# nv-tlabs/GEN3C

Measured on NVIDIA H100. Metric: denoise-steps/sec, 7B DiT, 121-frame 720p latent, higher is better.
Workload: dtype bf16

## Files before the change

gen3c_b200/csrc/attn_wgmma.cu:

```cuda
#include <cmath>
#include <cstdlib>

#include "kernels.h"

namespace g3c {

constexpr int ATT_THREADS = 384;
constexpr int ATT_TILE = ATT_ROWS_PER_CTA;
constexpr int ATT_HALF_BYTES = 128 * 128;
constexpr int ATT_TILE_BYTES = 2 * ATT_HALF_BYTES;
constexpr int ATT_STAGES = 2;
constexpr int ATT_SMEM = ATT_TILE_BYTES + ATT_STAGES * 2 * ATT_TILE_BYTES + 256 + 1024;
static_assert(ATT_SMEM <= 227 * 1024, "attention: Q + K/V rings exceed the 227 KB of shared memory per block");
static_assert(1 + 4 * ATT_STAGES + 3 <= 256 / 8, "attention: barriers exceed their 256-byte area");
static_assert(ATT_STAGES == 2, "attention: the consumer loop is unrolled for a ring depth of 2");
constexpr float ATT_RESCALE_LOG2 = 8.0f;

struct AttnParams {
  int Lq, Lk, heads;
  int ldo;
  int vt_chunk_len;
  __nv_bfloat16* O;
  float scale_log2;
  const uint32_t* chunk_flags;
  uint32_t flag_seq;
  int first_chunk;
  unsigned long long peer_timeout_ns;
  unsigned long long* wait_ns;
  unsigned long long* trace;
};

static unsigned long long* g_attn_trace = nullptr;

#define ATT_TR(role, slot)                                                                                  \
  do {                                                                                                      \
    if constexpr (kTrace) {                                                                                 \
      if (blockIdx.x == 0 && blockIdx.y == 0 && j < 64 && (threadIdx.x % 128) == 0)                         \
        p.trace[((role) * 64 + j) * 8 + (slot)] = clock64();                                                \
    }                                                                                                       \
  } while (0)

__device__ __forceinline__ float ex2_approx(float x) {
  float y;
  asm("ex2.approx.ftz.f32 %0, %1;\n" : "=f"(y) : "f"(x));
  return y;
}

__device__ __forceinline__ bool softmax_tile(float (&s)[64], float (&m_ref)[2], float (&l_run)[2], float (&alpha)[2],
                                             float sl2) {
  float mx[2] = {-INFINITY, -INFINITY};
#pragma unroll
  for (int i = 0; i < 16; ++i) {
    mx[0] = fmaxf(mx[0], fmaxf(s[4 * i], s[4 * i + 1]));
    mx[1] = fmaxf(mx[1], fmaxf(s[4 * i + 2], s[4 * i + 3]));
  }
#pragma unroll
  for (int h = 0; h < 2; ++h) {
    mx[h] = fmaxf(mx[h], __shfl_xor_sync(0xffffffffu, mx[h], 1));
    mx[h] = fmaxf(mx[h], __shfl_xor_sync(0xffffffffu, mx[h], 2));
    mx[h] *= sl2;
  }
  const bool keep = __all_sync(0xffffffffu, mx[0] - m_ref[0] <= ATT_RESCALE_LOG2 && mx[1] - m_ref[1] <= ATT_RESCALE_LOG2);
  if (!keep) {
#pragma unroll
    for (int h = 0; h < 2; ++h) {
      const float nm = fmaxf(m_ref[h], mx[h]);
      alpha[h] = ex2_approx(m_ref[h] - nm);
      m_ref[h] = nm;
      l_run[h] *= alpha[h];
    }
  }
  const float nm0 = -m_ref[0], nm1 = -m_ref[1];
#pragma unroll
  for (int i = 0; i < 16; ++i) {
    s[4 * i] = ex2_approx(fmaf(s[4 * i], sl2, nm0));
    s[4 * i + 1] = ex2_approx(fmaf(s[4 * i + 1], sl2, nm0));
    s[4 * i + 2] = ex2_approx(fmaf(s[4 * i + 2], sl2, nm1));
    s[4 * i + 3] = ex2_approx(fmaf(s[4 * i + 3], sl2, nm1));
    l_run[0] += s[4 * i] + s[4 * i + 1];
    l_run[1] += s[4 * i + 2] + s[4 * i + 3];
  }
  return !keep;
}

constexpr uint32_t ATT_SDESC_HI = (1024u >> 4) | (1u << 30);
__device__ __forceinline__ uint64_t sdesc_at(uint32_t lo, uint32_t bytes) {
  return (static_cast<uint64_t>(ATT_SDESC_HI) << 32) | (lo + (bytes >> 4));
}

__device__ __forceinline__ void issue_s(float (&s)[64], uint32_t dq, uint32_t dk) {
#pragma unroll
  for (int kk = 0; kk < 8; ++kk) {
    const uint32_t off = (kk >> 2) * ATT_HALF_BYTES + (kk & 3) * 32;
    wgmma_ss_n128(s, sdesc_at(dq, off), sdesc_at(dk, off), kk > 0 ? 1u : 0u);
  }
}

template <bool kVTokenMajor>
__device__ __forceinline__ void issue_pv(float (&o)[64], const uint32_t (&pa)[32], uint32_t dv) {
#pragma unroll
  for (int kk = 0; kk < 8; ++kk) {
    const uint32_t a[4] = {pa[4 * kk], pa[4 * kk + 1], pa[4 * kk + 2], pa[4 * kk + 3]};
    if constexpr (kVTokenMajor)
      wgmma_rs_n128_tb(o, a, sdesc_at(dv, kk * 16 * 128));
    else
      wgmma_rs_n128(o, a, sdesc_at(dv, (kk >> 2) * ATT_HALF_BYTES + (kk & 3) * 32));
  }
}

__device__ __forceinline__ void mask_key_tail(float (&s)[64], int valid, uint32_t lane) {
#pragma unroll
  for (int i = 0; i < 16; ++i) {
    const int col = 8 * i + 2 * (int)(lane % 4);
    if (col >= valid) s[4 * i] = s[4 * i + 2] = -INFINITY;
    if (col + 1 >= valid) s[4 * i + 1] = s[4 * i + 3] = -INFINITY;
  }
}

__device__ __forceinline__ void pack_p(uint32_t (&pa)[32], const float (&s)[64]) {
#pragma unroll
  for (int i = 0; i < 16; ++i) {
    pa[2 * i] = pack_bf16x2(s[4 * i], s[4 * i + 1]);
    pa[2 * i + 1] = pack_bf16x2(s[4 * i + 2], s[4 * i + 3]);
  }
}

template <bool kTrace, bool kVTokenMajor = false>
__global__ void __launch_bounds__(ATT_THREADS, 1)
    k_attn_fwd(const __grid_constant__ CUtensorMap tmQ, const __grid_constant__ CUtensorMap tmK,
               const __grid_constant__ CUtensorMap tmV, const AttnParams p) {
  extern __shared__ uint8_t smem_raw[];
  uint8_t* smem = reinterpret_cast<uint8_t*>((reinterpret_cast<uintptr_t>(smem_raw) + 1023) &
                                             ~static_cast<uintptr_t>(1023));
  uint8_t* smem_q = smem;
  uint8_t* smem_k = smem + ATT_TILE_BYTES;
  uint8_t* smem_v = smem_k + ATT_STAGES * ATT_TILE_BYTES;
  uint64_t* bars = reinterpret_cast<uint64_t*>(smem_v + ATT_STAGES * ATT_TILE_BYTES);
  uint64_t* q_full = bars;
  uint64_t* k_full = bars + 1;
  uint64_t* v_full = k_full + ATT_STAGES;
  uint64_t* k_empty = v_full + ATT_STAGES;
  uint64_t* v_empty = k_empty + ATT_STAGES;
  uint64_t* turn = v_empty + ATT_STAGES;
  uint64_t* done = turn + 2;

  const uint32_t wg = threadIdx.x / 128;
  const uint32_t tid = threadIdx.x % 128;
  const int head = blockIdx.y;
  const int q0 = blockIdx.x * ATT_TILE;
  const int n_kv = kVTokenMajor ? (p.Lk + ATT_TILE - 1) / ATT_TILE : p.Lk / ATT_TILE;

  if (threadIdx.x == 0) {
    tma_prefetch_desc(&tmQ);
    tma_prefetch_desc(&tmK);
    tma_prefetch_desc(&tmV);
    mbar_init(q_full, 1);
    for (int i = 0; i < ATT_STAGES; ++i) {
      mbar_init(&k_full[i], 1);
      mbar_init(&v_full[i], 1);
      mbar_init(&k_empty[i], 2);
      mbar_init(&v_empty[i], 2);
    }
    for (int c = 0; c < 2; ++c) mbar_init(&turn[c], 4);
    for (int w = 0; w < 4; ++w) mbar_arrive(&turn[0]);
    mbar_init(done, 2);
    fence_barrier_init();
  }
  __syncthreads();

  if (wg == 0) {
    setmaxnreg_dec<24>();
    if (tid == 0) {
      mbar_expect_tx(q_full, ATT_TILE_BYTES);
      for (int h = 0; h < 2; ++h) tma_load_2d(smem_q + h * ATT_HALF_BYTES, &tmQ, q_full, head * 128 + h * 64, q0);
      const int tiles_per_chunk = p.vt_chunk_len / ATT_TILE;
      const int n_chunks = p.Lk / p.vt_chunk_len;
      uint32_t stage = 0, phase = 0;
      for (int j = 0; j < n_kv; ++j) {
        int chunk = 0, within = j;
        if constexpr (!kVTokenMajor) {
          chunk = p.first_chunk + j / tiles_per_chunk;
          if (chunk >= n_chunks) chunk -= n_chunks;
          within = j % tiles_per_chunk;
          if (p.chunk_flags && within == 0 && chunk != p.first_chunk) {
            uint32_t v, spins = 0;
            uint64_t t0 = 0;
            for (;;) {
              asm volatile("ld.acquire.sys.global.u32 %0, [%1];\n" : "=r"(v) : "l"(p.chunk_flags + chunk) : "memory");
              if ((int)(v - p.flag_seq) >= 0) break;
              if (t0 == 0) t0 = global_timer_ns();
              if ((++spins & 0x3FFu) == 0 && global_timer_ns() - t0 > p.peer_timeout_ns) asm volatile("trap;\n");
            }
            if (t0 != 0 && p.wait_ns) atomicAdd(p.wait_ns, (unsigned long long)(global_timer_ns() - t0));
            asm volatile("fence.proxy.async.global;\n" ::: "memory");
          }
        }
        const int kv0 = chunk * p.vt_chunk_len + within * ATT_TILE;
        mbar_wait_ns(&k_empty[stage], phase ^ 1, p.peer_timeout_ns);
        mbar_expect_tx(&k_full[stage], ATT_TILE_BYTES);
        for (int h = 0; h < 2; ++h)
          tma_load_2d(smem_k + stage * ATT_TILE_BYTES + h * ATT_HALF_BYTES, &tmK, &k_full[stage], head * 128 + h * 64,
                      kv0);
        mbar_wait_ns(&v_empty[stage], phase ^ 1, p.peer_timeout_ns);
        mbar_expect_tx(&v_full[stage], ATT_TILE_BYTES);
        for (int h = 0; h < 2; ++h) {
          if constexpr (kVTokenMajor)
            tma_load_2d(smem_v + stage * ATT_TILE_BYTES + h * ATT_HALF_BYTES, &tmV, &v_full[stage],
                        head * 128 + h * 64, kv0);
          else
            tma_load_3d(smem_v + stage * ATT_TILE_BYTES + h * ATT_HALF_BYTES, &tmV, &v_full[stage],
                        within * ATT_TILE + h * 64, head * 128, chunk);
        }
        if (++stage == ATT_STAGES) {
          stage = 0;
          phase ^= 1;
        }
      }
      mbar_wait_ns(done, 0, p.peer_timeout_ns);
    }
  } else {
    setmaxnreg_inc<240>();
    const uint32_t c = __shfl_sync(0xffffffffu, wg - 1, 0);
    const uint32_t warp = tid / 32, lane = tid % 32;
    const unsigned long long tmo = p.peer_timeout_ns;
    float o[64];
#pragma unroll
    for (int i = 0; i < 64; ++i) o[i] = 0.f;
    float s[64];
    uint32_t pa[32];
    float m_ref[2] = {-INFINITY, -INFINITY};
    float l_run[2] = {0.f, 0.f};
    float alpha[2];
    const float sl2 = p.scale_log2;
    const uint32_t dq = (uint32_t)make_sdesc_sw128(smem_u32(smem_q + c * 64 * 128));
    uint32_t dk[ATT_STAGES], dv[ATT_STAGES];
#pragma unroll
    for (int st = 0; st < ATT_STAGES; ++st) {
      dk[st] = (uint32_t)make_sdesc_sw128(smem_u32(smem_k + st * ATT_TILE_BYTES));
      dv[st] = (uint32_t)(kVTokenMajor ? make_sdesc_sw128_mn(smem_u32(smem_v + st * ATT_TILE_BYTES), ATT_HALF_BYTES)
                                       : make_sdesc_sw128(smem_u32(smem_v + st * ATT_TILE_BYTES)));
    }
    int j = 0;
    mbar_wait_ns_or_exit(q_full, 0, tmo);
    mbar_wait_ns_or_exit(&k_full[0], 0, tmo);
    mbar_wait_ns_or_exit(&turn[c], 0, tmo);
    ATT_TR(1 + c, 0);
    wgmma_fence();
    issue_s(s, dq, dk[0]);
    wgmma_commit();
    if (lane == 0) mbar_arrive(&turn[c ^ 1]);
    ATT_TR(1 + c, 1);
    wgmma_wait<0>();
    fence_regs(s);
    if (tid == 0) mbar_arrive(&k_empty[0]);
    ATT_TR(1 + c, 2);
    if constexpr (kVTokenMajor) {
      if (n_kv == 1) mask_key_tail(s, p.Lk, lane);
    }
    softmax_tile(s, m_ref, l_run, alpha, sl2);
    pack_p(pa, s);
    ATT_TR(1 + c, 3);
    auto step = [&](int kst, int vst, uint32_t kpar, uint32_t vpar, int valid) {
      mbar_wait_ns_or_exit(&k_full[kst], kpar, tmo);
      mbar_wait_ns_or_exit(&v_full[vst], vpar, tmo);
      mbar_wait_ns_or_exit(&turn[c], (uint32_t)j & 1u, tmo);
      ATT_TR(1 + c, 0);
      wgmma_fence();
      issue_s(s, dq, kst ? dk[1] : dk[0]);
      wgmma_commit();
      issue_pv<kVTokenMajor>(o, pa, vst ? dv[1] : dv[0]);
      wgmma_commit();
      if (lane == 0) mbar_arrive(&turn[c ^ 1]);
      ATT_TR(1 + c, 1);
      wgmma_wait<1>();
      fence_regs(s);
      if (tid == 0) mbar_arrive(&k_empty[kst]);
      ATT_TR(1 + c, 2);
      if (valid < ATT_TILE) mask_key_tail(s, valid, lane);
      const bool rescale = softmax_tile(s, m_ref, l_run, alpha, sl2);
      ATT_TR(1 + c, 3);
      wgmma_wait<0>();
      fence_regs(o);
      fence_regs(pa);
      if (tid == 0) mbar_arrive(&v_empty[vst]);
      ATT_TR(1 + c, 4);
      if (rescale) {
#pragma unroll
        for (int i = 0; i < 16; ++i) {
          o[4 * i] *= alpha[0];
          o[4 * i + 1] *= alpha[0];
          o[4 * i + 2] *= alpha[1];
          o[4 * i + 3] *= alpha[1];
        }
      }
      pack_p(pa, s);
    };
    const int j_end = kVTokenMajor ? n_kv - 1 : n_kv;
    uint32_t ph = 0;
    for (j = 1; j < j_end; ++j) {
      step(1, 0, ph, ph, ATT_TILE);
      if (++j == j_end) break;
      step(0, 1, ph ^ 1u, ph, ATT_TILE);
      ph ^= 1u;
    }
    if constexpr (kVTokenMajor) {
      if (n_kv > 1) {
        j = n_kv - 1;
        step(j & 1, (j - 1) & 1, ((uint32_t)j >> 1) & 1u, ((uint32_t)(j - 1) >> 1) & 1u, p.Lk - j * ATT_TILE);
      }
      j = n_kv;
    }
    const int vst = (n_kv - 1) & 1;
    mbar_wait_ns_or_exit(&v_full[vst], ((uint32_t)(n_kv - 1) >> 1) & 1u, tmo);
    mbar_wait_ns_or_exit(&turn[c], (uint32_t)n_kv & 1u, tmo);
    ATT_TR(1 + c, 0);
    wgmma_fence();
    issue_pv<kVTokenMajor>(o, pa, vst ? dv[1] : dv[0]);
    wgmma_commit();
    if (lane == 0) mbar_arrive(&turn[c ^ 1]);
    ATT_TR(1 + c, 1);
    wgmma_wait<0>();
    fence_regs(o);
    fence_regs(pa);
    if (tid == 0) mbar_arrive(&v_empty[vst]);
    ATT_TR(1 + c, 4);
    float inv[2];
#pragma unroll
    for (int h = 0; h < 2; ++h) {
      float l = l_run[h];
      l += __shfl_xor_sync(0xffffffffu, l, 1);
      l += __shfl_xor_sync(0xffffffffu, l, 2);
      inv[h] = 1.0f / l;
    }
    const int row_a = q0 + (int)(c * 64 + warp * 16 + lane / 4);
#pragma unroll
    for (int h = 0; h < 2; ++h) {
      const int row = row_a + 8 * h;
      if (row >= p.Lq) continue;
      __nv_bfloat16* dst = p.O + (size_t)row * p.ldo + head * 128 + 2 * (lane % 4);
#pragma unroll
      for (int i = 0; i < 16; ++i)
        *reinterpret_cast<uint32_t*>(dst + 8 * i) = pack_bf16x2(o[4 * i + 2 * h] * inv[h], o[4 * i + 2 * h + 1] * inv[h]);
    }
    if (tid == 0) mbar_arrive(done);
  }
}

static int make_tmap_tokens(CUtensorMap* m, const void* base, int rows, int heads, int ld) {
  uint64_t dims[2] = {(uint64_t)heads * 128, (uint64_t)rows}, str[1] = {(uint64_t)ld * 2};
  uint32_t box[2] = {64, 128};
  return make_tmap_bf16_sw128(m, base, 2, dims, str, box);
}

static float scale_log2(float scale) {
  const float s = scale * 1.4426950408889634f;
  return fabsf(s - 1.0f) < 1e-6f ? 1.0f : s;
}

int attn_fwd(const void* q, const void* k, const void* vt, void* o, int Lq, int Lk, int heads,
             int ldq, int ldk, int ldo, int vt_chunk_len, float scale, cudaStream_t st, const ChunkGate* gate) {
  G3C_REQUIRE(q && k && vt && o, "attn: null operand");
  G3C_REQUIRE(Lq > 0 && Lk > 0 && heads > 0, "attn: bad sizes");
  G3C_REQUIRE(Lk % ATT_TILE == 0, "attn: Lk=%d must be a multiple of 128", Lk);
  if (vt_chunk_len <= 0) vt_chunk_len = Lk;
  G3C_REQUIRE(Lk % vt_chunk_len == 0 && vt_chunk_len % ATT_TILE == 0,
              "attn: vt_chunk_len=%d must divide Lk=%d and be a multiple of 128", vt_chunk_len, Lk);
  G3C_REQUIRE(ldq % 8 == 0 && ldk % 8 == 0 && ldo % 8 == 0 && ldq >= heads * 128 &&
                  ldk >= heads * 128 && ldo >= heads * 128,
              "attn: leading dimensions must be >= heads*128 and multiples of 8");
  G3C_REQUIRE((reinterpret_cast<uintptr_t>(o) & 15) == 0, "attn: O must be 16-byte aligned");
  CUtensorMap tmQ, tmK, tmV;
  int rc = make_tmap_tokens(&tmQ, q, Lq, heads, ldq);
  if (rc) return rc;
  rc = make_tmap_tokens(&tmK, k, Lk, heads, ldk);
  if (rc) return rc;
  {
    const int chunks = Lk / vt_chunk_len;
    uint64_t dims[3] = {(uint64_t)vt_chunk_len, (uint64_t)heads * 128, (uint64_t)chunks};
    uint64_t str[2] = {(uint64_t)vt_chunk_len * 2, (uint64_t)vt_chunk_len * 2 * heads * 128};
    uint32_t box[3] = {64, 128, 1};
    rc = make_tmap_bf16_sw128(&tmV, vt, 3, dims, str, box);
    if (rc) return rc;
  }
  static bool configured = false;
  if (!configured) {
    G3C_CUDA(cudaFuncSetAttribute(k_attn_fwd<false>, cudaFuncAttributeMaxDynamicSharedMemorySize, ATT_SMEM));
    G3C_CUDA(cudaFuncSetAttribute(k_attn_fwd<true>, cudaFuncAttributeMaxDynamicSharedMemorySize, ATT_SMEM));
    configured = true;
  }
  AttnParams p;
  p.Lq = Lq;
  p.Lk = Lk;
  p.heads = heads;
  p.ldo = ldo;
  p.vt_chunk_len = vt_chunk_len;
  p.O = reinterpret_cast<__nv_bfloat16*>(o);
  p.scale_log2 = scale_log2(scale);
  p.chunk_flags = gate ? gate->flags : nullptr;
  p.peer_timeout_ns = gate ? peer_timeout_ns() : G3C_MBAR_TIMEOUT_NS;
  p.wait_ns = gate ? gate->wait_ns : nullptr;
  p.flag_seq = gate ? gate->seq : 0;
  p.first_chunk = gate ? gate->first : 0;
  p.trace = g_attn_trace;
  G3C_REQUIRE(p.first_chunk >= 0 && p.first_chunk < Lk / vt_chunk_len, "attn: first chunk %d out of range", p.first_chunk);
  dim3 grid((Lq + ATT_TILE - 1) / ATT_TILE, heads);
  if (g_attn_trace) k_attn_fwd<true><<<grid, ATT_THREADS, ATT_SMEM, st>>>(tmQ, tmK, tmV, p);
  else k_attn_fwd<false><<<grid, ATT_THREADS, ATT_SMEM, st>>>(tmQ, tmK, tmV, p);
  G3C_CUDA(cudaGetLastError());
  return G3C_OK;
}

int attn_fwd_sbhd(const void* q, const void* k, const void* v, void* o, int Lq, int Lk, int batch, int heads, int ldq,
                  int ldk, int ldv, int ldo, float scale, cudaStream_t st) {
  G3C_REQUIRE(q && k && v && o, "attn_sbhd: null operand");
  G3C_REQUIRE(Lq > 0 && Lk > 0, "attn_sbhd: Lq=%d and Lk=%d must be >= 1", Lq, Lk);
  G3C_REQUIRE(batch > 0 && heads > 0 && (long long)batch * heads <= 65535,
              "attn_sbhd: batch=%d x heads=%d must be in [1, 65535]", batch, heads);
  const int bh = batch * heads;
  G3C_REQUIRE(ldq % 8 == 0 && ldk % 8 == 0 && ldv % 8 == 0 && ldo % 8 == 0 && ldq >= bh * 128 && ldk >= bh * 128 &&
                  ldv >= bh * 128 && ldo >= bh * 128,
              "attn_sbhd: leading dimensions (%d, %d, %d, %d) must be >= batch*heads*128 = %d and multiples of 8", ldq,
              ldk, ldv, ldo, bh * 128);
  G3C_REQUIRE(((reinterpret_cast<uintptr_t>(q) | reinterpret_cast<uintptr_t>(k) | reinterpret_cast<uintptr_t>(v) |
                reinterpret_cast<uintptr_t>(o)) & 15) == 0,
              "attn_sbhd: q, k, v and o must be 16-byte aligned");
  CUtensorMap tmQ, tmK, tmV;
  int rc = make_tmap_tokens(&tmQ, q, Lq, bh, ldq);
  if (rc) return rc;
  rc = make_tmap_tokens(&tmK, k, Lk, bh, ldk);
  if (rc) return rc;
  rc = make_tmap_tokens(&tmV, v, Lk, bh, ldv);
  if (rc) return rc;
  static bool configured = false;
  if (!configured) {
    G3C_CUDA(cudaFuncSetAttribute(k_attn_fwd<false, true>, cudaFuncAttributeMaxDynamicSharedMemorySize, ATT_SMEM));
    configured = true;
  }
  AttnParams p = {};
  p.Lq = Lq;
  p.Lk = Lk;
  p.heads = bh;
  p.ldo = ldo;
  p.vt_chunk_len = Lk;
  p.O = reinterpret_cast<__nv_bfloat16*>(o);
  p.scale_log2 = scale_log2(scale);
  p.peer_timeout_ns = G3C_MBAR_TIMEOUT_NS;
  dim3 grid((Lq + ATT_TILE - 1) / ATT_TILE, bh);
  k_attn_fwd<false, true><<<grid, ATT_THREADS, ATT_SMEM, st>>>(tmQ, tmK, tmV, p);
  G3C_CUDA(cudaGetLastError());
  return G3C_OK;
}

}

extern "C" int g3c_attn_set_trace(unsigned long long* device_buffer) {
  g3c::g_attn_trace = device_buffer;
  return G3C_OK;
}

extern "C" int g3c_attn_fwd(const void* q, const void* k, const void* vt, void* o, int Lq, int Lk,
                            int heads, int ldq, int ldk, int ldo, int vt_chunk_len, float scale,
                            void* stream) {
  return g3c::attn_fwd(q, k, vt, o, Lq, Lk, heads, ldq, ldk, ldo, vt_chunk_len, scale,
                       (cudaStream_t)stream, nullptr);
}

extern "C" int g3c_attn_fwd_gated(const void* q, const void* k, const void* vt, void* o, int Lq, int Lk, int heads,
                                  int ldq, int ldk, int ldo, int vt_chunk_len, float scale, const uint32_t* flags,
                                  uint32_t seq, int first, unsigned long long* wait_ns, void* stream) {
  g3c::ChunkGate gate;
  gate.flags = flags;
  gate.seq = seq;
  gate.first = first;
  gate.wait_ns = wait_ns;
  return g3c::attn_fwd(q, k, vt, o, Lq, Lk, heads, ldq, ldk, ldo, vt_chunk_len, scale, (cudaStream_t)stream, &gate);
}

extern "C" int g3c_attn_fwd_sbhd(const void* q, const void* k, const void* v, void* o, int Lq, int Lk, int batch,
                                 int heads, int ldq, int ldk, int ldv, int ldo, float scale, void* stream) {
  return g3c::attn_fwd_sbhd(q, k, v, o, Lq, Lk, batch, heads, ldq, ldk, ldv, ldo, scale, (cudaStream_t)stream);
}
```

gen3c_b200/csrc/common.cuh:

```cuda
#pragma once
#include <cuda.h>
#include <cuda_bf16.h>
#include <cuda_runtime.h>
#include <stdint.h>
#include <stdio.h>

#include "../../include/gen3c_b200.h"
#include "wgmma_ops.cuh"

namespace g3c {

void set_error(const char* fmt, ...);
int cuda_fail(cudaError_t e, const char* what, const char* file, int line);
#define G3C_CUDA(x)                                                         \
  do {                                                                      \
    cudaError_t _e = (x);                                                   \
    if (_e != cudaSuccess) return ::g3c::cuda_fail(_e, #x, __FILE__, __LINE__); \
  } while (0)
#define G3C_REQUIRE(cond, ...)        \
  do {                                \
    if (!(cond)) {                    \
      ::g3c::set_error(__VA_ARGS__);  \
      return G3C_EINVAL;       \
    }                                 \
  } while (0)

int make_tmap_bf16_sw128(CUtensorMap* out, const void* base, int rank, const uint64_t* dims,
                         const uint64_t* strides_bytes, const uint32_t* box,
                         CUtensorMapDataType dtype = CU_TENSOR_MAP_DATA_TYPE_BFLOAT16);
int make_tmap_f32_sw128(CUtensorMap* out, const void* base, const uint64_t* dims,
                        const uint64_t* strides_bytes, const uint32_t* box);

int sm_count();

#ifdef __CUDACC__
__device__ __forceinline__ uint32_t smem_u32(const void* p) {
  return static_cast<uint32_t>(__cvta_generic_to_shared(p));
}
__device__ __forceinline__ uint32_t lane_id() { return threadIdx.x & 31; }
__device__ __forceinline__ uint32_t warp_id() { return __shfl_sync(0xffffffffu, threadIdx.x >> 5, 0); }

__device__ __forceinline__ bool elect_one() {
  uint32_t pred = 0;
  asm volatile(
      "{\n\t.reg .pred P;\n\t"
      "elect.sync _|P, 0xffffffff;\n\t"
      "selp.b32 %0, 1, 0, P;\n\t}\n"
      : "=r"(pred));
  return pred != 0;
}

__device__ __forceinline__ void mbar_init(uint64_t* bar, uint32_t count) {
  asm volatile("mbarrier.init.shared::cta.b64 [%0], %1;\n" ::"r"(smem_u32(bar)), "r"(count));
}
__device__ __forceinline__ void fence_barrier_init() {
  asm volatile("fence.mbarrier_init.release.cluster;\n" ::: "memory");
}
__device__ __forceinline__ void fence_proxy_async() {
  asm volatile("fence.proxy.async.shared::cta;\n" ::: "memory");
}
__device__ __forceinline__ void mbar_expect_tx(uint64_t* bar, uint32_t bytes) {
  asm volatile("mbarrier.arrive.expect_tx.shared::cta.b64 _, [%0], %1;\n" ::"r"(smem_u32(bar)),
               "r"(bytes)
               : "memory");
}
__device__ __forceinline__ void mbar_arrive(uint64_t* bar) {
  asm volatile("mbarrier.arrive.shared::cta.b64 _, [%0];\n" ::"r"(smem_u32(bar)) : "memory");
}
#ifndef G3C_MBAR_SUSPEND_NS
#define G3C_MBAR_SUSPEND_NS 0
#endif
__device__ __forceinline__ bool mbar_try_wait(uint64_t* bar, uint32_t parity) {
  uint32_t ok;
#if G3C_MBAR_SUSPEND_NS > 0
  asm volatile(
      "{\n\t.reg .pred P;\n\t"
      "mbarrier.try_wait.parity.shared::cta.b64 P, [%1], %2, %3;\n\t"
      "selp.b32 %0, 1, 0, P;\n\t}\n"
      : "=r"(ok)
      : "r"(smem_u32(bar)), "r"(parity), "r"((uint32_t)G3C_MBAR_SUSPEND_NS)
      : "memory");
#else
  asm volatile(
      "{\n\t.reg .pred P;\n\t"
      "mbarrier.try_wait.parity.shared::cta.b64 P, [%1], %2;\n\t"
      "selp.b32 %0, 1, 0, P;\n\t}\n"
      : "=r"(ok)
      : "r"(smem_u32(bar)), "r"(parity)
      : "memory");
#endif
  return ok != 0;
}
__device__ __forceinline__ bool mbar_test(uint64_t* bar, uint32_t parity) {
  uint32_t ok;
  asm volatile(
      "{\n\t.reg .pred P;\n\t"
      "mbarrier.test_wait.parity.shared::cta.b64 P, [%1], %2;\n\t"
      "selp.b32 %0, 1, 0, P;\n\t}\n"
      : "=r"(ok)
      : "r"(smem_u32(bar)), "r"(parity)
      : "memory");
  return ok != 0;
}
#ifndef G3C_MBAR_TIMEOUT_NS
#define G3C_MBAR_TIMEOUT_NS 4000000000ull
#endif
__device__ __forceinline__ uint64_t global_timer_ns() {
  uint64_t t;
  asm volatile("mov.u64 %0, %%globaltimer;\n" : "=l"(t));
  return t;
}
#ifdef G3C_MBAR_DEBUG
#define G3C_MBAR_TIMEOUT_ACTION(bar, parity)                                                                 \
  do {                                                                                                       \
    printf("g3c: mbarrier timeout block(%d,%d) thread %d bar@%u parity %u\n", blockIdx.x, blockIdx.y,        \
           threadIdx.x, bar, parity);                                                                        \
    __trap();                                                                                                \
  } while (0)
#else
#define G3C_MBAR_TIMEOUT_ACTION(bar, parity) asm volatile("trap;\n")
#endif
__device__ __forceinline__ void mbar_wait(uint64_t* bar, uint32_t parity) {
  if (mbar_try_wait(bar, parity)) return;
  uint32_t spins = 0;
  uint64_t t0 = 0;
  while (!mbar_try_wait(bar, parity)) {
    if ((++spins & 0xFFFu) == 0) {
      uint64_t now = global_timer_ns();
      if (t0 == 0) t0 = now;
      else if (now - t0 > G3C_MBAR_TIMEOUT_NS) G3C_MBAR_TIMEOUT_ACTION(smem_u32(bar), parity);
    }
  }
}

__device__ __forceinline__ void mbar_wait_ns(uint64_t* bar, uint32_t parity, unsigned long long timeout_ns) {
  if (mbar_try_wait(bar, parity)) return;
  uint32_t spins = 0;
  uint64_t t0 = 0;
  while (!mbar_try_wait(bar, parity)) {
    if ((++spins & 0xFFFu) == 0) {
      uint64_t now = global_timer_ns();
      if (t0 == 0) t0 = now;
      else if (now - t0 > timeout_ns) G3C_MBAR_TIMEOUT_ACTION(smem_u32(bar), parity);
    }
  }
}

__device__ __forceinline__ void mbar_wait_ns_or_exit(uint64_t* bar, uint32_t parity, unsigned long long timeout_ns) {
  if (mbar_try_wait(bar, parity)) return;
  uint32_t spins = 0;
  uint64_t t0 = 0;
  while (!mbar_try_wait(bar, parity)) {
    if ((++spins & 0xFFFu) == 0) {
      uint64_t now = global_timer_ns();
      if (t0 == 0) t0 = now;
      else if (now - t0 > timeout_ns) asm volatile("exit;\n");
    }
  }
}

__device__ __forceinline__ void tma_prefetch_desc(const CUtensorMap* m) {
  asm volatile("prefetch.tensormap [%0];\n" ::"l"(reinterpret_cast<uint64_t>(m)) : "memory");
}
__device__ __forceinline__ void tma_load_2d(void* smem_dst, const CUtensorMap* m, uint64_t* bar,
                                            int c0, int c1) {
  asm volatile(
      "cp.async.bulk.tensor.2d.shared::cluster.global.mbarrier::complete_tx::bytes"
      " [%0], [%1, {%3, %4}], [%2];\n" ::"r"(smem_u32(smem_dst)),
      "l"(reinterpret_cast<uint64_t>(m)), "r"(smem_u32(bar)), "r"(c0), "r"(c1)
      : "memory");
}
__device__ __forceinline__ void tma_load_3d(void* smem_dst, const CUtensorMap* m, uint64_t* bar,
                                            int c0, int c1, int c2) {
  asm volatile(
      "cp.async.bulk.tensor.3d.shared::cluster.global.mbarrier::complete_tx::bytes"
      " [%0], [%1, {%3, %4, %5}], [%2];\n" ::"r"(smem_u32(smem_dst)),
      "l"(reinterpret_cast<uint64_t>(m)), "r"(smem_u32(bar)), "r"(c0), "r"(c1), "r"(c2)
      : "memory");
}

__device__ __forceinline__ void tma_store_2d(const CUtensorMap* m, const void* smem_src, int c0, int c1) {
  asm volatile("cp.async.bulk.tensor.2d.global.shared::cta.bulk_group [%0, {%2, %3}], [%1];\n" ::"l"(
                   reinterpret_cast<uint64_t>(m)),
               "r"(smem_u32(smem_src)), "r"(c0), "r"(c1)
               : "memory");
}
__device__ __forceinline__ void tma_reduce_add_2d(const CUtensorMap* m, const void* smem_src, int c0, int c1) {
  asm volatile("cp.reduce.async.bulk.tensor.2d.global.shared::cta.add.bulk_group [%0, {%2, %3}], [%1];\n" ::"l"(
                   reinterpret_cast<uint64_t>(m)),
               "r"(smem_u32(smem_src)), "r"(c0), "r"(c1)
               : "memory");
}
__device__ __forceinline__ void tma_store_commit() { asm volatile("cp.async.bulk.commit_group;\n" ::: "memory"); }
template <int N>
__device__ __forceinline__ void tma_store_wait_read() {
  asm volatile("cp.async.bulk.wait_group.read %0;\n" ::"n"(N) : "memory");
}
template <int N>
__device__ __forceinline__ void tma_store_wait_all() {
  asm volatile("cp.async.bulk.wait_group %0;\n" ::"n"(N) : "memory");
}

__device__ __forceinline__ void wgmma_fence() { asm volatile("wgmma.fence.sync.aligned;\n" ::: "memory"); }
__device__ __forceinline__ void wgmma_commit() { asm volatile("wgmma.commit_group.sync.aligned;\n" ::: "memory"); }
template <int N>
__device__ __forceinline__ void wgmma_wait() {
  asm volatile("wgmma.wait_group.sync.aligned %0;\n" ::"n"(N) : "memory");
}
template <int N>
__device__ __forceinline__ void fence_regs(float (&r)[N]) {
#pragma unroll
  for (int i = 0; i < N; ++i) asm volatile("" : "+f"(r[i])::"memory");
}
template <int N>
__device__ __forceinline__ void fence_regs(uint32_t (&r)[N]) {
#pragma unroll
  for (int i = 0; i < N; ++i) asm volatile("" : "+r"(r[i])::"memory");
}

__device__ __forceinline__ uint64_t make_sdesc_sw128(uint32_t smem_addr) {
  uint64_t d = 0;
  d |= static_cast<uint64_t>((smem_addr & 0x3FFFFu) >> 4);
  d |= static_cast<uint64_t>(1) << 16;
  d |= static_cast<uint64_t>(1024u >> 4) << 32;
  d |= static_cast<uint64_t>(1) << 62;
  return d;
}
__device__ __forceinline__ uint64_t make_sdesc_sw128_mn(uint32_t smem_addr, uint32_t mn_block_bytes) {
  uint64_t d = 0;
  d |= static_cast<uint64_t>((smem_addr & 0x3FFFFu) >> 4);
  d |= static_cast<uint64_t>((mn_block_bytes >> 4) & 0x3FFFu) << 16;
  d |= static_cast<uint64_t>(1024u >> 4) << 32;
  d |= static_cast<uint64_t>(1) << 62;
  return d;
}
__device__ __forceinline__ uint64_t sdesc_advance(uint64_t d, uint32_t bytes) {
  return d + static_cast<uint64_t>(bytes >> 4);
}

template <int N>
__device__ __forceinline__ void setmaxnreg_dec() {
  asm volatile("setmaxnreg.dec.sync.aligned.u32 %0;\n" ::"n"(N));
}
template <int N>
__device__ __forceinline__ void setmaxnreg_inc() {
  asm volatile("setmaxnreg.inc.sync.aligned.u32 %0;\n" ::"n"(N));
}

__device__ __forceinline__ uint32_t pack_bf16x2(float lo, float hi) {
  __nv_bfloat162 v = __floats2bfloat162_rn(lo, hi);
  return *reinterpret_cast<uint32_t*>(&v);
}
__device__ __forceinline__ float warp_max(float v) {
#pragma unroll
  for (int o = 16; o > 0; o >>= 1) v = fmaxf(v, __shfl_xor_sync(0xffffffffu, v, o));
  return v;
}
__device__ __forceinline__ float warp_sum(float v) {
#pragma unroll
  for (int o = 16; o > 0; o >>= 1) v += __shfl_xor_sync(0xffffffffu, v, o);
  return v;
}
#endif

}
```

Measured before the change: 0.1372.

## Speculatively exponentiate scores against stale max, recompute QK^T on overflow

The consumer loop no longer computes a row max before exponentiating. It applies exp2 directly with the previous running max and checks the per-row sums against a large guard using a warpgroup barrier reduction. If the guard trips, it reissues the QK^T wgmma, waits for it, and runs the full max-based softmax. The release of the K buffer moves to after that decision so the retry can still read K. This removes the max reduction and its shuffles from the common path, but adds a named barrier per tile, delays the K-slot release, and risks precision loss, since values up to the guard can be accumulated without rescaling.

Result: faster. 0.1432, median of 6 (+4.4%).

```diff
diff --git a/gen3c_b200/csrc/attn_wgmma.cu b/gen3c_b200/csrc/attn_wgmma.cu
--- a/gen3c_b200/csrc/attn_wgmma.cu
+++ b/gen3c_b200/csrc/attn_wgmma.cu
@@ -15,6 +15,7 @@
 static_assert(1 + 4 * ATT_STAGES + 3 <= 256 / 8, "attention: barriers exceed their 256-byte area");
 static_assert(ATT_STAGES == 2, "attention: the consumer loop is unrolled for a ring depth of 2");
 constexpr float ATT_RESCALE_LOG2 = 8.0f;
+constexpr float ATT_GUARD = 16777216.0f;
 
 struct AttnParams {
   int Lq, Lk, heads;
@@ -46,6 +47,19 @@
   return y;
 }
 
+__device__ __forceinline__ void exp_tile(float (&s)[64], const float (&m_ref)[2], float (&acc)[2], float sl2) {
+  const float nm0 = -m_ref[0], nm1 = -m_ref[1];
+#pragma unroll
+  for (int i = 0; i < 16; ++i) {
+    s[4 * i] = ex2_approx(fmaf(s[4 * i], sl2, nm0));
+    s[4 * i + 1] = ex2_approx(fmaf(s[4 * i + 1], sl2, nm0));
+    s[4 * i + 2] = ex2_approx(fmaf(s[4 * i + 2], sl2, nm1));
+    s[4 * i + 3] = ex2_approx(fmaf(s[4 * i + 3], sl2, nm1));
+    acc[0] += s[4 * i] + s[4 * i + 1];
+    acc[1] += s[4 * i + 2] + s[4 * i + 3];
+  }
+}
+
 __device__ __forceinline__ bool softmax_tile(float (&s)[64], float (&m_ref)[2], float (&l_run)[2], float (&alpha)[2],
                                              float sl2) {
   float mx[2] = {-INFINITY, -INFINITY};
@@ -70,16 +84,7 @@
       l_run[h] *= alpha[h];
     }
   }
-  const float nm0 = -m_ref[0], nm1 = -m_ref[1];
-#pragma unroll
-  for (int i = 0; i < 16; ++i) {
-    s[4 * i] = ex2_approx(fmaf(s[4 * i], sl2, nm0));
-    s[4 * i + 1] = ex2_approx(fmaf(s[4 * i + 1], sl2, nm0));
-    s[4 * i + 2] = ex2_approx(fmaf(s[4 * i + 2], sl2, nm1));
-    s[4 * i + 3] = ex2_approx(fmaf(s[4 * i + 3], sl2, nm1));
-    l_run[0] += s[4 * i] + s[4 * i + 1];
-    l_run[1] += s[4 * i + 2] + s[4 * i + 3];
-  }
+  exp_tile(s, m_ref, l_run, sl2);
   return !keep;
 }
 
@@ -274,10 +279,27 @@
       ATT_TR(1 + c, 1);
       wgmma_wait<1>();
       fence_regs(s);
-      if (tid == 0) mbar_arrive(&k_empty[kst]);
       ATT_TR(1 + c, 2);
       if (valid < ATT_TILE) mask_key_tail(s, valid, lane);
-      const bool rescale = softmax_tile(s, m_ref, l_run, alpha, sl2);
+      float t[2] = {0.f, 0.f};
+      exp_tile(s, m_ref, t, sl2);
+      const bool redo = bar_red_or(1 + c, 128, !(t[0] < ATT_GUARD && t[1] < ATT_GUARD));
+      if (redo) {
+        wgmma_fence();
+        issue_s(s, dq, kst ? dk[1] : dk[0]);
+        wgmma_commit();
+        wgmma_wait<0>();
+        fence_regs(s);
+      }
+      if (tid == 0) mbar_arrive(&k_empty[kst]);
+      bool rescale = false;
+      if (redo) {
+        if (valid < ATT_TILE) mask_key_tail(s, valid, lane);
+        rescale = softmax_tile(s, m_ref, l_run, alpha, sl2);
+      } else {
+        l_run[0] += t[0];
+        l_run[1] += t[1];
+      }
       ATT_TR(1 + c, 3);
       wgmma_wait<0>();
       fence_regs(o);
diff --git a/gen3c_b200/csrc/common.cuh b/gen3c_b200/csrc/common.cuh
--- a/gen3c_b200/csrc/common.cuh
+++ b/gen3c_b200/csrc/common.cuh
@@ -159,6 +159,19 @@
   }
 }
 
+__device__ __forceinline__ bool bar_red_or(uint32_t id, uint32_t nthreads, bool pred) {
+  uint32_t r;
+  asm volatile(
+      "{\n\t.reg .pred P, Q;\n\t"
+      "setp.ne.u32 P, %1, 0;\n\t"
+      "bar.red.or.pred Q, %2, %3, P;\n\t"
+      "selp.u32 %0, 1, 0, Q;\n\t}\n"
+      : "=r"(r)
+      : "r"((uint32_t)pred), "r"(id), "r"(nthreads)
+      : "memory");
+  return r != 0;
+}
+
 __device__ __forceinline__ void tma_prefetch_desc(const CUtensorMap* m) {
   asm volatile("prefetch.tensormap [%0];\n" ::"l"(reinterpret_cast<uint64_t>(m)) : "memory");
 }
```
